# MrGreyPanda/NEM-MCMC-optimization

Hardware: AMD Instinct MI355X
Metric: order-score evals/sec (64 S-genes x 2000 effects); HBM GB/s fraction (higher is better)
Workload: dtype int8 fixed point 2^-38/ln2 + fp64 LSE

## Files before the change

### nem-mcmc-optimization_amd/csrc/nemo_factored_i8.hip

```cpp
#include "nemo_internal.h"

#include <math.h>

#include <string.h>

#include <algorithm>
#include <cmath>
#include <vector>

#ifndef NEMO_I8_ABLATE
#define NEMO_I8_ABLATE 0
#endif
#ifndef NEMO_I8L_RINIT
#define NEMO_I8L_RINIT 1
#endif
#ifndef NEMO_I8L_CINIT16
#define NEMO_I8L_CINIT16 1
#endif
#ifndef NEMO_I8L_PINGPONG
#define NEMO_I8L_PINGPONG 1
#endif
#ifndef NEMO_I8_WAVES_PER_SIMD
#define NEMO_I8_WAVES_PER_SIMD 2
#endif

namespace nemo {

namespace {

using i32x4 = __attribute__((ext_vector_type(4))) int;

constexpr double kPadG8 = -1.0e6;
constexpr int kARow = 6;
template <int ROWC>
__device__ __forceinline__ int a_byte(int i, int j) {
  if constexpr (ROWC == 4) return i * 64 + (((j >> 4) + 2 * ((i >> 2) & 3)) & 3) * 16 + (j & 15);
  else return i * (16 * ROWC) + j;
}

__device__ __forceinline__ double wsum(double v) {
#pragma unroll
  for (int o = 32; o >= 1; o >>= 1) v += __shfl_xor(v, o, kWave);
  return v;
}

__device__ __forceinline__ double exp_lse8(double x, const double* __restrict__ tab) {
  constexpr double kInvLn2x256 = 369.32993046757462707;
  constexpr double kLn2d256 = 2.7076061740622862e-03;
  constexpr double kMagic = 6755399441055744.0;
  const double t = fma(x, kInvLn2x256, kMagic);
  const double kf = t - kMagic;
  const int k = (int)(uint32_t)__builtin_bit_cast(uint64_t, t);
  const double r = fma(-kf, kLn2d256, x);
  double p = fma(r, 1.0 / 24.0, 1.0 / 6.0);
  p = fma(r, p, 0.5);
  p = fma(r, p, 1.0);
  p = fma(r, p, 1.0);
  return ldexp(p * tab[k & 255], k >> 8);
}

__device__ __forceinline__ double vmax8(double a, double b) {
  double r;
  asm("v_max_f64 %0, %1, %2" : "=v"(r) : "v"(a), "v"(b));
  return r;
}

__device__ __forceinline__ int xcd_index8(int L, int N, int remap) {
  if (!remap) return L;
  const int x = L & 7, k = L >> 3;
  const int q = N >> 3, r = N & 7;
  return x * q + (x < r ? x : r) + k;
}

struct EvalLds {
  i32x4* A;
  double* G;
  int* perm;
};

constexpr int kExpTabN = 2048;
constexpr int kTabBytes = kExpTabN * 8 + 128 * 16;

template <int SPAD, int NSL, int KH = 1, int NBUF = 1>
struct I8Lds {
  static constexpr int kElo = kTabBytes, kEhi = kElo + SPAD * 8, kBuf0 = kEhi + SPAD * 8;
  static constexpr int kG = 0, kGi = SPAD * 8, kPerm = kGi + 2 * SPAD * 4, kA = kPerm + SPAD * 4;
  static constexpr int kABytes = NSL * KH * SPAD * 64, kBuf = kA + kABytes, kImg = kBuf - kGi;
  static constexpr int kBytes = kBuf0 + NBUF * kBuf;
  static_assert((kBuf0 + kGi) % 16 == 0 && kA % 16 == 0 && kBuf % 16 == 0, "16-B alignment of gi and A");
  static_assert(NSL != 7 || KH != 1 || kImg == SPAD * kI8ImgRowBytes, "i8img_bytes follows this layout");

  static constexpr size_t bytes(size_t a_min = 0) {
    return (size_t)kBytes + (a_min > (size_t)kABytes ? a_min - kABytes : 0);
  }
  static __device__ __forceinline__ double2* ltab(double* lds) { return (double2*)((char*)lds + kExpTabN * 8); }
  static __device__ __forceinline__ double* elo(double* lds) { return (double*)((char*)lds + kElo); }
  static __device__ __forceinline__ double* ehi(double* lds) { return (double*)((char*)lds + kEhi); }
  static __device__ __forceinline__ EvalLds eval(double* lds, int k = 0) {
    char* p = (char*)lds + kBuf0 + k * kBuf;
    return EvalLds{(i32x4*)(p + kA), (double*)(p + kG), (int*)(p + kPerm)};
  }
  static __device__ __forceinline__ int* gi(double* lds, int k = 0) {
    return (int*)((char*)lds + kBuf0 + k * kBuf + kGi);
  }
};

template <int SPAD, int NSL, int ROWC = kARow>
__device__ __forceinline__ void i8_init_eval(EvalLds e, const int32_t* __restrict__ pb, int S, int tid,
                                             int nthreads, double padg = kPadG8) {
  for (int j = tid; j < S; j += nthreads) {
    int pj = pb[j];
    pj = pj < 0 ? 0 : (pj >= S ? S - 1 : pj);
    e.perm[pj] = j;
  }
  for (int i = tid; i < SPAD; i += nthreads) e.G[i] = i < S ? 0.0 : padg;
  for (int k = tid; k < NSL * SPAD * ROWC; k += nthreads) e.A[k] = i32x4{0, 0, 0, 0};
}

__device__ __forceinline__ int i8_npass(int S, int cap) {
  return (cap == 0 || cap >= S - 1) ? (S + 1) / 2 : S;
}

template <int WAVES>
__device__ __forceinline__ int i8_wave_passes(int S, int cap, int w) {
  const int npass = i8_npass(S, cap);
  return npass > w ? (npass - w + WAVES - 1) / WAVES : 0;
}

template <int SPAD, int NSL, int WAVES, int KB, int ROWC = kARow>
__device__ __forceinline__ void i8_prep_passes(EvalLds e, int k0, int w, int lane, int S, int cap,
                                               int cexp, const double* __restrict__ w01b,
                                               const double* __restrict__ elo_s,
                                               const double* __restrict__ ehi_s,
                                               const double2* __restrict__ ltab) {
  const bool packed = cap == 0 || cap >= S - 1;
  const int npass = packed ? (S + 1) / 2 : S;
  const int p = lane;
  int8_t* A8 = (int8_t*)e.A;
  int ii[KB], jj[KB];
  double sw[KB], ga[KB], gb[KB];
#pragma unroll
  for (int kk = 0; kk < KB; ++kk) {
    const int q = w + (k0 + kk) * WAVES;
    int qr = 0, pp = 0;
    bool act = false;
    if (q < npass) {
      if (packed) {
        const int q2 = S - 1 - q;
        if (p < q) { qr = q; pp = p; act = true; }
        else { qr = q2; pp = p - q; act = q2 != q && pp < q2; }
      } else {
        const int np = q < cap ? q : cap;
        qr = q; pp = q - 1 - p; act = p < np;
      }
    }
    ii[kk] = act ? e.perm[qr] : -1;
    jj[kk] = act ? e.perm[pp] : 0;
    sw[kk] = act ? w01b[ii[kk] * S + jj[kk]] : 0.0;
  }
#pragma unroll
  for (int kk = 0; kk < KB; ++kk) {
    const int q = w + (k0 + kk) * WAVES;
    const bool act = ii[kk] >= 0;
    double lo = 0.0;
    if (act && !(NEMO_I8_ABLATE & 8)) {
      const int i = ii[kk], j = jj[kk];
      const double s1 = 1.0 - sw[kk];
      lo = log_fast(fma(sw[kk], elo_s[j], s1), ltab);
      const double d = log_fast(fma(sw[kk], ehi_s[j], s1), ltab) - lo;
      double x = ldexp(d, 6 - cexp);
#pragma unroll
      for (int sl = 0; sl < NSL; ++sl) {
        const double qd = rint(x);
// ... 512 lines not shown
  constexpr int NP = 4;
  constexpr int NSL = 2 * NP;
  using L = I8Lds<SPAD, NSL>;
  extern __shared__ __attribute__((aligned(16))) double lds8[];
  const uint2* etab_o = (const uint2*)lds8;
  double2* ltab = L::ltab(lds8);
  double *elo_s = L::elo(lds8), *ehi_s = L::ehi(lds8);
  const EvalLds ev = L::eval(lds8);
  int* gi = L::gi(lds8);

  const I8Block blk = i8_block(nsets, split, remap);
  const int b = blk.b, s_begin = blk.s_begin, s_end = blk.s_end;
  const int tid = threadIdx.x;
  const int lane = tid & (kWave - 1);
  const int w = __builtin_amdgcn_readfirstlane(tid / kWave);
  const int col = lane & 15, rg = lane >> 4;

  i8_copy_tables<SPAD>(lds8, elo_s, ehi_s, tabs, e_lo, e_hi, S, tid, blockDim.x);
  i8_init_eval<SPAD, NSL, 4>(ev, pos + (size_t)b * S, S, tid, blockDim.x, padg);
  __syncthreads();
  if constexpr (DIAG) {
    int8_t* A8 = (int8_t*)ev.A;
    for (int k = tid; k < S * NSL; k += blockDim.x) {
      const int i = k / NSL, sl = k - i * NSL;
      A8[sl * SPAD * 64 + a_byte<4>(i, i)] = udig[k];
    }
  }
  for (int k0 = 0, my = i8_wave_passes<WAVES>(S, cap, w); k0 < my; k0 += 4)
    i8o_prep_passes<SPAD, WAVES, 4, 4>(ev, k0, w, lane, S, cap, cexp, w01 + (size_t)b * S * S, elo_s,
                                       ehi_s, ltab);
  __syncthreads();
  for (int i = tid; i < SPAD; i += blockDim.x) {
    const double g = DIAG && i < S ? ev.G[i] + u0[i] : ev.G[i];
    const double g0 = rint(ldexp(g, 24 - cexp));
    const double rho = fma(-g0, ldexp(1.0, cexp - 24), g);
    gi[i] = (int)g0;
    gi[SPAD + i] = (int)rint(ldexp(rho, 48 - cexp));
  }
  const uint32_t uln8 = (uint32_t)(4 * rg * E + col) * 8u;
  __syncthreads();
#if NEMO_I8_ABLATE & 32
  if (s_end > 0) return;
#endif

  const i32x4* Bt = (const i32x4*)B8;
  const i32x4* Gi = (const i32x4*)gi;
  const uint32_t a_lane = (uint32_t)(col * 4 + ((rg + 2 * (col >> 2)) & 3));
  int set = s_begin + w;
  if (set < s_end) {
    double lprod = 1.0;
    int lexp = 0;
    double uc[NR][4];
    int t = 8 * set;
    const __amdgpu_buffer_rsrc_t urs =
        __builtin_amdgcn_make_buffer_rsrc((void*)Uoff, (short)0, (int)((SPAD + 1) * E + 16) * 8, 0x00020000);
    auto uload = [&](int tt, int row) {
      return __builtin_bit_cast(double, __builtin_amdgcn_raw_buffer_load_b64(
                                            urs, uln8, (tt * 16 + row * E) * 8, 0));
    };
    if constexpr (!DIAG)
#pragma unroll
      for (int r = 0; r < NR; ++r)
#pragma unroll
        for (int g = 0; g < 4; ++g) uc[r][g] = uload(t, 16 * r + g);
    i32x4 bc = Bt[(size_t)t * kWave + lane];
    for (;;) {
      uint32_t ao = a_lane;
      asm volatile("" : "+v"(ao));
      const i32x4* Al = ev.A + ao;
      int tn = t + 1, setn = set;
      if (tn >= min(ntiles, 8 * set + 8)) {
        setn = set + WAVES;
        tn = 8 * setn;
      }
      const bool more = setn < s_end;
      const int tl = more ? tn : t;
      const i32x4 b1 = bc;
      const i32x4 b64 = b1 << 6;
      bc = Bt[(size_t)tl * kWave + lane];
      double ls0 = 0.0, ls1 = 0.0;
#pragma unroll
      for (int r = 0; r < NR; ++r) {
        i32x4 acc[NP];
        const i32x4 c0 = Gi[(16 * r) / 4 + rg];
        const i32x4 c1 = Gi[(SPAD + 16 * r) / 4 + rg];
#pragma unroll
        for (int pr = 0; pr < NP; ++pr) {
          const i32x4 a0 = Al[((2 * pr) * SPAD + 16 * r) * 4];
          const i32x4 a1 = Al[((2 * pr + 1) * SPAD + 16 * r) * 4];
          const i32x4 ci = pr == 1 ? c0 : (pr == 3 ? c1 : i32x4{0, 0, 0, 0});
          acc[pr] = __builtin_amdgcn_mfma_i32_16x16x64_i8(a0, b64, ci, 0, 0, 0);
          acc[pr] = __builtin_amdgcn_mfma_i32_16x16x64_i8(a1, b1, acc[pr], 0, 0, 0);
        }
#pragma unroll
        for (int g = 0; g < 4; ++g) {
          const int ta = (acc[0][g] << 12) + acc[1][g];
          const int tb = (acc[2][g] << 12) + acc[3][g];
          double x;
          if constexpr (DIAG) {
            x = fma((double)ta, sA, (double)tb * sB);
          } else {
            x = fma((double)ta, sA, fma((double)tb, sB, uc[r][g]));
            uc[r][g] = uload(tl, 16 * r + g);
          }
#if NEMO_I8_ABLATE & 1
          if (g & 1) ls1 += x;
          else ls0 += x;
#else
          if (g & 1) ls1 = exp_acc(x, etab_o, ls1);
          else ls0 = exp_acc(x, etab_o, ls0);
#endif
        }
      }
      i8_colprod(lprod, lexp, rowsum4(ls0 + ls1) + 1.0, t * 16 + col < E);
      if (setn != set) {
        double v = log(lprod) + (double)lexp * kLn2;
        v = wsum(lane < 16 ? v : 0.0);
        if (lane == 0) partial[(size_t)b * nsets + set] = nullsum[set] + v;
        lprod = 1.0;
        lexp = 0;
      }
      if (!more) break;
      t = tn;
      set = setn;
    }
  }
  if (split == 1) {
    __syncthreads();
    if (w == 0) {
      const double v = sum_partials(partial + (size_t)b * nsets, nsets, lane);
      if (lane == 0) ll_out[b] = v;
    }
  }
}

template <int NR, int WAVES, bool DIAG>
hipError_t launch_i8o_t(Ctx& c, int batch, int cap, const int32_t* d_pos, const double* d_w01,
                        double* d_ll, hipStream_t st, int* nparts, bool* finalized) {
  constexpr int SPAD = NR * 16;
  const int ntiles = (c.E + 15) / 16;
  const int nsets = (ntiles + 7) / 8;
  const int split = i8_split(256 * (NEMO_I8O_WAVES_PER_SIMD * 4 / WAVES), batch, nsets);
  const size_t lds = I8Lds<SPAD, 8>::bytes();
  const double sA = ldexp(1.0, c.i8_cexp - 24), sB = ldexp(1.0, c.i8_cexp - 48);
  score_i8o_kernel<NR, WAVES, DIAG><<<dim3(batch * split), WAVES * kWave, lds, st>>>(
      c.S, c.E, ntiles, nsets, split, cap, c.i8_cexp, c.i8o_padg, d_pos, d_w01, c.d_elo, c.d_ehi,
      c.d_B8, c.d_Uoff, c.d_udig, c.d_u0, c.d_nullsum, c.d_i8o_tabs, sA, sB, fpartial(c), d_ll,
      c.xcd_remap);
  *nparts = nsets;
  *finalized = split == 1;
  return hipGetLastError();
}

template <int NR, int WAVES, bool PP, class Hook>
__device__ __forceinline__ int i8l_walk2(const i32x4* __restrict__ Al0, const i32x4* __restrict__ Gi,
                                        const i32x4* __restrict__ Bt, const i32x4* __restrict__ Bt64,
                                        int set, int s_end, int ntiles, int E, int col, int lane,
                                        uint32_t a_lane, const double* __restrict__ nullsum,
                                        double* __restrict__ partial, size_t b, int nsets,
                                        const double2* __restrict__ ltab, Hook hook) {
  constexpr int SPAD = NR * 16;
  const int rg = lane >> 4;
  int it = 0;
  if (set < s_end) {
    double lprod = 1.0;
    int lexp = 0;
    int t = 8 * set;
    auto tend = [&](int st) { return min(ntiles, 8 * st + 8); };
    int t2 = t + 1 < tend(set) ? t + 1 : t;
    const __amdgpu_buffer_rsrc_t brs =
        __builtin_amdgcn_make_buffer_rsrc((void*)Bt, (short)0, 2 * ntiles * kWave * 16, 0x00020000);
    const uint32_t bln = (uint32_t)lane * 16u;
    auto bload = [&](int tile, int x64) {
      return __builtin_bit_cast(i32x4, __builtin_amdgcn_raw_buffer_load_b128(
                                           brs, bln, (x64 * ntiles + tile) * kWave * 16, 0));
    };
    i32x4 bca = bload(t, 0), bca64 = bload(t, 1);
    i32x4 bcb = bload(t2, 0), bcb64 = bload(t2, 1);
    auto iter = [&](const i32x4 b1a, const i32x4 b64a, const i32x4 b1b, const i32x4 b64b, i32x4& na,
                    i32x4& na64, i32x4& nb, i32x4& nb64) -> bool {
      uint32_t ao = a_lane;
      asm volatile("" : "+v"(ao));
      const i32x4* Al = Al0 + ao;
      const bool two = t2 != t;
      int tn = t + 2, setn = set;
      if (tn >= tend(set)) {
        setn = set + WAVES;
        tn = 8 * setn;
      }
      const bool more = setn < s_end;
      const int tla = __builtin_amdgcn_readfirstlane(more ? tn : t);
      const int tlb = __builtin_amdgcn_readfirstlane(more ? (tn + 1 < tend(setn) ? tn + 1 : tn) : t);
      na = bload(tla, 0);
      na64 = bload(tla, 1);
      nb = bload(tlb, 0);
      nb64 = bload(tlb, 1);
      double la0 = 0.0, la1 = 0.0, lb0 = 0.0, lb1 = 0.0;
#pragma unroll
      for (int r = 0; r < NR; ++r) {
        const i32x4 c0 = Gi[(16 * r) / 4 + rg];
        const i32x4 c1 = Gi[(SPAD + 16 * r) / 4 + rg];
        auto A = [&](int sl) { return Al[(sl * SPAD + 16 * r) * 4]; };
        i32x4 h0a, h0b, h1a, h1b, l0a, l0b, l1a, l1b;
        {
          const i32x4 a = A(0);
          h0a = __builtin_amdgcn_mfma_i32_16x16x64_i8(a, b64a, i32x4{0, 0, 0, 0}, 0, 0, 0);
          h0b = __builtin_amdgcn_mfma_i32_16x16x64_i8(a, b64b, i32x4{0, 0, 0, 0}, 0, 0, 0);
        }
        {
          const i32x4 a = A(1);
          h0a = __builtin_amdgcn_mfma_i32_16x16x64_i8(a, b1a, h0a, 0, 0, 0);
          h0b = __builtin_amdgcn_mfma_i32_16x16x64_i8(a, b1b, h0b, 0, 0, 0);
        }
        {
          const i32x4 a = A(2);
          h1a = __builtin_amdgcn_mfma_i32_16x16x64_i8(a, b64a, c0, 0, 0, 0);
          h1b = __builtin_amdgcn_mfma_i32_16x16x64_i8(a, b64b, c0, 0, 0, 0);
        }
        {
          const i32x4 a = A(3);
          h1a = __builtin_amdgcn_mfma_i32_16x16x64_i8(a, b1a, h1a, 0, 0, 0);
          h1b = __builtin_amdgcn_mfma_i32_16x16x64_i8(a, b1b, h1b, 0, 0, 0);
        }
#if NEMO_I8L_RINIT
        {
          const i32x4 a = A(5);
          l1a = __builtin_amdgcn_mfma_i32_16x16x64_i8(a, b64a, c1, 0, 0, 0);
          l1b = __builtin_amdgcn_mfma_i32_16x16x64_i8(a, b64b, c1, 0, 0, 0);
        }
        {
          const i32x4 a = A(6);
          l1a = __builtin_amdgcn_mfma_i32_16x16x64_i8(a, b1a, l1a, 0, 0, 0);
          l1b = __builtin_amdgcn_mfma_i32_16x16x64_i8(a, b1b, l1b, 0, 0, 0);
        }
        uint32_t t0a[4], t0b[4];
        uint64_t eva[4], evb[4];
        i32x4 ma, mb;
#pragma unroll
        for (int g = 0; g < 4; ++g) {
          t0a[g] = ((uint32_t)h0a[g] << 12) + (uint32_t)h1a[g];
          eva[g] = exp2_fx_load(t0a[g]);
          ma[g] = i8l_cinit16(t0a[g]);
        }
#pragma unroll
        for (int g = 0; g < 4; ++g) {
          t0b[g] = ((uint32_t)h0b[g] << 12) + (uint32_t)h1b[g];
          evb[g] = exp2_fx_load(t0b[g]);
          mb[g] = i8l_cinit16(t0b[g]);
        }
        {
          const i32x4 a = A(4);
          l0a = __builtin_amdgcn_mfma_i32_16x16x64_i8(a, b1a, ma, 0, 0, 0);
          l0b = __builtin_amdgcn_mfma_i32_16x16x64_i8(a, b1b, mb, 0, 0, 0);
        }
        auto epi = [&](const uint32_t (&t0)[4], const uint64_t (&evv)[4], const i32x4 l0, const i32x4 l1,
                       double& ls0, double& ls1) {
          double pr[4];
#pragma unroll
          for (int g = 0; g < 4; ++g) pr[g] = exp2_fx_series_r((int)(((uint32_t)l0[g] << 11) + (uint32_t)l1[g]));
#pragma unroll
          for (int g = 0; g < 4; ++g) {
            if (g & 1) ls1 = exp2_fx_apply(t0[g], evv[g], pr[g], ls1);
            else ls0 = exp2_fx_apply(t0[g], evv[g], pr[g], ls0);
          }
        };
        epi(t0a, eva, l0a, l1a, la0, la1);
        epi(t0b, evb, l0b, l1b, lb0, lb1);
#else
        {
          const i32x4 a = A(4);
          l0a = __builtin_amdgcn_mfma_i32_16x16x64_i8(a, b1a, i32x4{0, 0, 0, 0}, 0, 0, 0);
          l0b = __builtin_amdgcn_mfma_i32_16x16x64_i8(a, b1b, i32x4{0, 0, 0, 0}, 0, 0, 0);
        }
        {
          const i32x4 a = A(5);
          l1a = __builtin_amdgcn_mfma_i32_16x16x64_i8(a, b64a, c1, 0, 0, 0);
          l1b = __builtin_amdgcn_mfma_i32_16x16x64_i8(a, b64b, c1, 0, 0, 0);
        }
        {
          const i32x4 a = A(6);
          l1a = __builtin_amdgcn_mfma_i32_16x16x64_i8(a, b1a, l1a, 0, 0, 0);
          l1b = __builtin_amdgcn_mfma_i32_16x16x64_i8(a, b1b, l1b, 0, 0, 0);
        }
        auto epi = [&](const i32x4 h0, const i32x4 h1, const i32x4 l0, const i32x4 l1, double& ls0,
                       double& ls1) {
          uint32_t t0[4];
          uint64_t evv[4];
          double pr[4];
#pragma unroll
          for (int g = 0; g < 4; ++g) {
            t0[g] = ((uint32_t)h0[g] << 12) + (uint32_t)h1[g];
            evv[g] = exp2_fx_load(t0[g]);
          }
#pragma unroll
          for (int g = 0; g < 4; ++g)
            pr[g] = exp2_fx_series(t0[g], (int)(((uint32_t)l0[g] << 11) + (uint32_t)l1[g]));
#pragma unroll
          for (int g = 0; g < 4; ++g) {
            if (g & 1) ls1 = exp2_fx_apply(t0[g], evv[g], pr[g], ls1);
            else ls0 = exp2_fx_apply(t0[g], evv[g], pr[g], ls0);
          }
        };
        epi(h0a, h1a, l0a, l1a, la0, la1);
        epi(h0b, h1b, l0b, l1b, lb0, lb1);
#endif
      }
      const double l = rowsum_pair(la0 + la1, lb0 + lb1) + 1.0;
      const bool tb = (lane & 16) != 0;
      const bool ok = (((tb ? t2 : t) * 16 + col) < E) & (two | !tb);
      i8_colprod(lprod, lexp, l, ok);
      if (setn != set) {
        i8l_set_finish<true>(lprod, lexp, ltab, lane, nullsum, partial, b, nsets, set);
        lprod = 1.0;
        lexp = 0;
      }
      hook(it++);
      if (!more) return false;
      t = tn;
      t2 = tlb;
      set = setn;
      return true;
    };
    if constexpr (PP) {
      i32x4 bqa, bqa64, bqb, bqb64;
      for (;;) {
        if (!iter(bca, bca64, bcb, bcb64, bqa, bqa64, bqb, bqb64)) break;
        if (!iter(bqa, bqa64, bqb, bqb64, bca, bca64, bcb, bcb64)) break;
      }
    } else {
      for (;;) {
        i32x4 na, na64, nb, nb64;
        const bool more = iter(bca, bca64, bcb, bcb64, na, na64, nb, nb64);
        bca = na;
        bca64 = na64;
        bcb = nb;
        bcb64 = nb64;
        if (!more) break;
      }
    }
  }
  return it;
}

template <int NR, int WAVES, int OCC, int TT = 1, int MODE = 0>
__global__ __launch_bounds__(WAVES * kWave, OCC) void score_i8l_kernel(
    int S, int E, int ntiles, int nsets, int split, int cap, double padg,
    const int32_t* __restrict__ pos, const double* __restrict__ w01,
    const double* __restrict__ e_lo, const double* __restrict__ e_hi,
    const uint8_t* __restrict__ B8, const int8_t* __restrict__ udig, const double* __restrict__ u0,
    const double* __restrict__ nullsum, const void* __restrict__ tabs,
    double* __restrict__ partial, double* __restrict__ ll_out, int remap,
    int4* __restrict__ img = nullptr) {
  constexpr int SPAD = NR * 16;
  constexpr int NSL = 7;
  using L = I8Lds<SPAD, NSL>;
  extern __shared__ __attribute__((aligned(16))) double lds8[];
  double2* ltab = L::ltab(lds8);
  double *elo_s = L::elo(lds8), *ehi_s = L::ehi(lds8);
  const EvalLds ev = L::eval(lds8);
  int* gi = L::gi(lds8);

  const int work = xcd_index8((int)blockIdx.x, (int)gridDim.x, remap);
  const int b = work / split;
  const int part = work - b * split;
  const int spb = (nsets + split - 1) / split;
  const int s_begin = part * spb;
  const int s_end = min(nsets, s_begin + spb);
  const int tid = threadIdx.x;
  const int lane = tid & (kWave - 1);
  const int w = __builtin_amdgcn_readfirstlane(tid / kWave);
  const int col = lane & 15, rg = lane >> 4;

  constexpr int kImg4 = L::kImg / 16;
  {
    const int4* src = (const int4*)tabs;
    int4* dst = (int4*)lds8;
    for (int k = tid + (MODE == 1 ? kExpTabN * 8 / 16 : 0); k < kTabBytes / 16; k += blockDim.x)
      dst[k] = src[k];
    if constexpr (MODE != 2)
      for (int i = tid; i < SPAD; i += blockDim.x) {
        elo_s[i] = i < S ? e_lo[i] : 1.0;
        ehi_s[i] = i < S ? e_hi[i] : 1.0;
      }
  }
  if constexpr (MODE == 2) {
    const int4* src = img + (size_t)b * kImg4;
    int4* dst = (int4*)gi;
    for (int k = tid; k < kImg4; k += blockDim.x) dst[k] = src[k];
    __syncthreads();
  } else {
    i8_init_eval<SPAD, NSL, 4>(ev, pos + (size_t)b * S, S, tid, blockDim.x, padg);
    __syncthreads();
    i8l_diag<SPAD>(ev.A, udig, S, tid, blockDim.x);
    for (int k0 = 0, my = i8_wave_passes<WAVES>(S, cap, w); k0 < my; k0 += 4)
      i8o_prep_passes<SPAD, WAVES, 4, 4, true>(ev, k0, w, lane, S, cap, 0, w01 + (size_t)b * S * S, elo_s,
                                               ehi_s, ltab);
    __syncthreads();
    i8l_split_g<SPAD>(ev, gi, u0, S, tid, blockDim.x);
    __syncthreads();
    if constexpr (MODE == 1) {
      const int4* src = (const int4*)gi;
      int4* dst = img + (size_t)b * kImg4;
      for (int k = tid; k < kImg4; k += blockDim.x) dst[k] = src[k];
      return;
    }
  }
#if NEMO_I8_ABLATE & 32
  if (s_end > 0) return;
#endif

  const i32x4* Bt = (const i32x4*)B8;
  const i32x4* Bt64 = Bt + (size_t)ntiles * kWave;
  const i32x4* Gi = (const i32x4*)gi;
  const uint32_t a_lane = (uint32_t)(col * 4 + ((rg + 2 * (col >> 2)) & 3));
  int set = s_begin + w;
  if constexpr (TT == 1) {
    int set = s_begin + w;
    if (set < s_end) {
      double lprod = 1.0;
      int lexp = 0;
      int t = 8 * set;
      i32x4 bc = Bt[(size_t)t * kWave + lane];
      i32x4 bc64 = Bt64[(size_t)t * kWave + lane];
      for (;;) {
        uint32_t ao = a_lane;
        asm volatile("" : "+v"(ao));
        const i32x4* Al = ev.A + ao;
        int tn = t + 1, setn = set;
        if (tn >= min(ntiles, 8 * set + 8)) {
          setn = set + WAVES;
          tn = 8 * setn;
        }
        const bool more = setn < s_end;
        const int tl = more ? tn : t;
        const i32x4 b1 = bc, b64 = bc64;
        bc = Bt[(size_t)tl * kWave + lane];
        bc64 = Bt64[(size_t)tl * kWave + lane];
        double ls0 = 0.0, ls1 = 0.0;
  #pragma unroll
        for (int r = 0; r < NR; ++r) {
          const i32x4 c0 = Gi[(16 * r) / 4 + rg];
          const i32x4 c1 = Gi[(SPAD + 16 * r) / 4 + rg];
  #if NEMO_I8_ABLATE & 128
          auto A = [&](int sl) { return Al[((sl & ~1) * SPAD + 16 * r) * 4]; };
  #else
          auto A = [&](int sl) { return Al[(sl * SPAD + 16 * r) * 4]; };
  #endif
  #if NEMO_I8_ABLATE & 2
          const i32x4 h0 = A(0) + A(1) + b64, h1 = A(2) + A(3) + c0, l0 = A(4) + b1,
                      l1 = A(5) + A(6) + c1;
  #else
          i32x4 h0 = __builtin_amdgcn_mfma_i32_16x16x64_i8(A(0), b64, i32x4{0, 0, 0, 0}, 0, 0, 0);
          h0 = __builtin_amdgcn_mfma_i32_16x16x64_i8(A(1), b1, h0, 0, 0, 0);
          i32x4 h1 = __builtin_amdgcn_mfma_i32_16x16x64_i8(A(2), b64, c0, 0, 0, 0);
          h1 = __builtin_amdgcn_mfma_i32_16x16x64_i8(A(3), b1, h1, 0, 0, 0);
          const i32x4 l0 = __builtin_amdgcn_mfma_i32_16x16x64_i8(A(4), b1, i32x4{0, 0, 0, 0}, 0, 0, 0);
          i32x4 l1 = __builtin_amdgcn_mfma_i32_16x16x64_i8(A(5), b64, c1, 0, 0, 0);
          l1 = __builtin_amdgcn_mfma_i32_16x16x64_i8(A(6), b1, l1, 0, 0, 0);
  #endif
          uint32_t t0[4];
          uint64_t evv[4];
          double pr[4];
#pragma unroll
          for (int g = 0; g < 4; ++g) {
            t0[g] = ((uint32_t)h0[g] << 12) + (uint32_t)h1[g];
            evv[g] = exp2_fx_load(t0[g]);
          }
#pragma unroll
          for (int g = 0; g < 4; ++g)
            pr[g] = exp2_fx_series(t0[g], (int)(((uint32_t)l0[g] << 11) + (uint32_t)l1[g]));
#pragma unroll
          for (int g = 0; g < 4; ++g) {
            if (g & 1) ls1 = exp2_fx_apply(t0[g], evv[g], pr[g], ls1);
            else ls0 = exp2_fx_apply(t0[g], evv[g], pr[g], ls0);
          }
        }
        i8_colprod(lprod, lexp, rowsum4(ls0 + ls1) + 1.0, t * 16 + col < E);
        if (setn != set) {
          i8l_set_finish<false>(lprod, lexp, ltab, lane, nullsum, partial, b, nsets, set);
          lprod = 1.0;
          lexp = 0;
        }
        if (!more) break;
        t = tn;
        set = setn;
      }
    }
  } else {
    i8l_walk2<NR, WAVES, NEMO_I8L_PINGPONG != 0>(ev.A, Gi, Bt, Bt64, set, s_end, ntiles, E, col, lane, a_lane,
                                                 nullsum, partial, b, nsets, ltab, [](int) {});
  }
  if (split == 1) {
    __syncthreads();
    if (w == 0) {
      const double v = sum_partials(partial + (size_t)b * nsets, nsets, lane);
      if (lane == 0) ll_out[b] = v;
    }
  }
}

constexpr size_t kI8sColsum = 16384;

template <int NR>
__global__ __launch_bounds__(8 * kWave, NEMO_I8O_WAVES_PER_SIMD) void score_i8s_kernel(
    int S, int E, int ntiles, int nsets, int split, int cap, double padg,
    const int32_t* __restrict__ pos, const double* __restrict__ w01,
    const double* __restrict__ e_lo, const double* __restrict__ e_hi,
    const uint8_t* __restrict__ B8, const int8_t* __restrict__ udig, const double* __restrict__ u0,
    const double* __restrict__ nullsum, const void* __restrict__ tabs,
    double* __restrict__ partial, double* __restrict__ ll_out, int remap) {
  constexpr int WAVES = 8;
  constexpr int SPAD = NR * 16;
  constexpr int NSL = 7;
  constexpr int NG = WAVES / NR;
  using L = I8Lds<SPAD, NSL>;
  extern __shared__ __attribute__((aligned(16))) double lds8[];
  double2* ltab = L::ltab(lds8);
  double *elo_s = L::elo(lds8), *ehi_s = L::ehi(lds8);
  const EvalLds ev = L::eval(lds8);
  int* gi = L::gi(lds8);
  double* colsum = (double*)ev.A;

  const I8Block blk = i8_block(nsets, split, remap);
  const int b = blk.b, s_begin = blk.s_begin, s_end = blk.s_end;
  const int tid = threadIdx.x;
  const int lane = tid & (kWave - 1);
  const int w = __builtin_amdgcn_readfirstlane(tid / kWave);
  const int rb = w % NR, grp = w / NR;
  const int col = lane & 15, rg = lane >> 4;

  i8_copy_tables<SPAD>(lds8, elo_s, ehi_s, tabs, e_lo, e_hi, S, tid, blockDim.x);
  i8_init_eval<SPAD, NSL, 4>(ev, pos + (size_t)b * S, S, tid, blockDim.x, padg);
  __syncthreads();
  i8l_diag<SPAD>(ev.A, udig, S, tid, blockDim.x);
  for (int k0 = 0, my = i8_wave_passes<WAVES>(S, cap, w); k0 < my; k0 += 4)
    i8o_prep_passes<SPAD, WAVES, 4, 4, true>(ev, k0, w, lane, S, cap, 0, w01 + (size_t)b * S * S, elo_s,
                                             ehi_s, ltab);
  __syncthreads();
  i8l_split_g<SPAD>(ev, gi, u0, S, tid, blockDim.x);
  __syncthreads();
  i32x4 af[NSL];
  {
    const i32x4* Al = ev.A + (uint32_t)(col * 4 + ((rg + 2 * (col >> 2)) & 3));
#pragma unroll
    for (int sl = 0; sl < NSL; ++sl) af[sl] = Al[(sl * SPAD + 16 * rb) * 4];
  }
  const i32x4 c0 = ((const i32x4*)gi)[(16 * rb) / 4 + rg];
  const i32x4 c1 = ((const i32x4*)gi)[(SPAD + 16 * rb) / 4 + rg];
  __syncthreads();
#if NEMO_I8_ABLATE & 32
  if (s_end > 0) return;
#endif

  const i32x4* Bt = (const i32x4*)B8;
  const int nsb = s_end > s_begin ? s_end - s_begin : 0;
  const int niter = (nsb + NG - 1) / NG;
  int tpre = 8 * (s_begin + grp);
  i32x4 bc = Bt[(size_t)min(tpre, ntiles - 1) * kWave + lane];
  for (int k = 0; k < niter; ++k) {
    const int set = s_begin + k * NG + grp;
    double* cs = colsum + (size_t)((grp * 2 + (k & 1)) * 8) * NR * 16;
    if (set < s_end) {
      const int t_end = min(ntiles, 8 * set + 8);
      for (int t = 8 * set; t < t_end; ++t) {
        const int tn = t + 1 < t_end ? t + 1 : 8 * (set + NG);
        const i32x4 b1 = bc;
        const i32x4 b64 = b1 << 6;
        bc = Bt[(size_t)min(tn, ntiles - 1) * kWave + lane];
        const i32x4 h0 = __builtin_amdgcn_mfma_i32_16x16x64_i8(
            af[1], b1, __builtin_amdgcn_mfma_i32_16x16x64_i8(af[0], b64, i32x4{0, 0, 0, 0}, 0, 0, 0), 0, 0, 0);
        const i32x4 h1 = __builtin_amdgcn_mfma_i32_16x16x64_i8(
            af[3], b1, __builtin_amdgcn_mfma_i32_16x16x64_i8(af[2], b64, c0, 0, 0, 0), 0, 0, 0);
        const i32x4 l0 = __builtin_amdgcn_mfma_i32_16x16x64_i8(af[4], b1, i32x4{0, 0, 0, 0}, 0, 0, 0);
        const i32x4 l1 = __builtin_amdgcn_mfma_i32_16x16x64_i8(
            af[6], b1, __builtin_amdgcn_mfma_i32_16x16x64_i8(af[5], b64, c1, 0, 0, 0), 0, 0, 0);
        double ls0 = 0.0, ls1 = 0.0;
        uint32_t t0[4];
        uint64_t evt[4];
        double pr[4];
#pragma unroll
        for (int g = 0; g < 4; ++g) {
          t0[g] = ((uint32_t)h0[g] << 12) + (uint32_t)h1[g];
          evt[g] = exp2_fx_load(t0[g]);
        }
#pragma unroll
        for (int g = 0; g < 4; ++g)
          pr[g] = exp2_fx_series(t0[g], (int)(((uint32_t)l0[g] << 11) + (uint32_t)l1[g]));
#pragma unroll
        for (int g = 0; g < 4; ++g) {
          if (g & 1) ls1 = exp2_fx_apply(t0[g], evt[g], pr[g], ls1);
          else ls0 = exp2_fx_apply(t0[g], evt[g], pr[g], ls0);
        }
        const double v = rowsum4(ls0 + ls1);
        if (lane < 16) cs[((t - 8 * set) * NR + rb) * 16 + col] = v;
      }
    }
    __syncthreads();
    if (set < s_end && rb == k % NR) {
      double lp = 1.0;
      int le = 0;
#pragma unroll
      for (int h = 0; h < 2; ++h) {
        const int tt = (lane >> 4) + 4 * h;
        const int t = 8 * set + tt;
        double l = 1.0;
#pragma unroll
        for (int q = 0; q < NR; ++q) l += cs[(tt * NR + q) * 16 + col];
        i8_colprod(lp, le, l, t < ntiles && t * 16 + col < E);
      }
      const double v = wsum(log(lp) + (double)le * kLn2);
      if (lane == 0) partial[(size_t)b * nsets + set] = nullsum[set] + v;
    }
  }
  if (split == 1) {
    __syncthreads();
    if (w == 0) {
      const double v = sum_partials(partial + (size_t)b * nsets, nsets, lane);
      if (lane == 0) ll_out[b] = v;
    }
  }
}

template <int NR, int WAVES>
__global__ __launch_bounds__(WAVES * kWave, NEMO_I8L2_OCC) void score_i8p_kernel(
    int S, int E, int ntiles, int nsets, int batch, int cap, double padg,
    const int32_t* __restrict__ pos, const double* __restrict__ w01,
    const double* __restrict__ e_lo, const double* __restrict__ e_hi,
    const uint8_t* __restrict__ B8, const int8_t* __restrict__ udig, const double* __restrict__ u0,
    const double* __restrict__ nullsum, const void* __restrict__ tabs,
    double* __restrict__ partial, double* __restrict__ ll_out) {
  constexpr int SPAD = NR * 16;
  constexpr int NSL = 7;
  constexpr int kBufG = 0, kBufGi = SPAD * 8, kBufPerm = kBufGi + 2 * SPAD * 4, kBufA = kBufPerm + SPAD * 4;
  constexpr int kBuf = kBufA + NSL * SPAD * 64;
  static_assert(kBuf == I8Lds<SPAD, NSL, 1, 2>::kBuf && kBufA == I8Lds<SPAD, NSL>::kA, "I8Lds describes it");
  extern __shared__ __attribute__((aligned(16))) double lds8[];
  uint2* etab_o = (uint2*)lds8;
  double2* ltab = (double2*)(etab_o + kExpTabN);
  double* elo_s = (double*)(ltab + 128);
  double* ehi_s = elo_s + SPAD;
  char* bufs = (char*)(ehi_s + SPAD);
  auto evb = [&](int k) {
    EvalLds e;
    char* p = bufs + k * kBuf;
    e.G = (double*)(p + kBufG);
    e.perm = (int*)(p + kBufPerm);
    e.A = (i32x4*)(p + kBufA);
    return e;
  };
  auto gib = [&](int k) { return (int*)(bufs + k * kBuf + kBufGi); };

  const int tid = threadIdx.x;
  const int lane = tid & (kWave - 1);
  const int w = __builtin_amdgcn_readfirstlane(tid / kWave);
  const int col = lane & 15, rg = lane >> 4;
  const int nb = gridDim.x;
  const int b0 = blockIdx.x;
  if (b0 >= batch) return;

  auto set_perm = [&](int k, int e) {
    int* perm = evb(k).perm;
    for (int j = tid; j < S; j += blockDim.x) {
      int pj = pos[(size_t)e * S + j];
      pj = pj < 0 ? 0 : (pj >= S ? S - 1 : pj);
      perm[pj] = j;
    }
  };
  auto zero_a = [&](int k) {
    i32x4* A = evb(k).A;
    for (int q = tid; q < NSL * SPAD * 4; q += blockDim.x) A[q] = i32x4{0, 0, 0, 0};
  };
  auto diag = [&](int k) {
    int8_t* A8 = (int8_t*)evb(k).A;
    for (int q = tid; q < S * NSL; q += blockDim.x) {
      const int i = q / NSL, sl = q - i * NSL;
      const int8_t d = udig[i * 8 + sl];
      A8[sl * SPAD * 64 + a_byte<4>(i, i)] = sl == 4 ? (int8_t)(2 * d) : d;
    }
  };
  auto prep = [&](int k, int e) {
    constexpr int KB = 4;
    const int npass = i8_npass(S, cap);
    const int my = npass > w ? (npass - w + WAVES - 1) / WAVES : 0;
    for (int k0 = 0; k0 < my; k0 += KB)
      i8o_prep_passes<SPAD, WAVES, KB, 4, true>(evb(k), k0, w, lane, S, cap, 0, w01 + (size_t)e * S * S,
                                                elo_s, ehi_s, ltab);
  };
  auto finalize_g = [&](int k) {
    const EvalLds ev = evb(k);
    int* gi = gib(k);
    for (int i = tid; i < SPAD; i += blockDim.x) {
      const double g = i < S ? ev.G[i] + u0[i] : ev.G[i];
      const double g0 = rint(g * kL2Scale);
      gi[i] = (int)g0 + (1023 << 20);
      gi[SPAD + i] = (int)rint(fma(g, kL2Scale, -g0) * 262144.0);
    }
  };

  {
    const int4* src = (const int4*)tabs;
    int4* dst = (int4*)lds8;
    for (int k = tid; k < (kExpTabN * 8 + 128 * 16) / 16; k += blockDim.x) dst[k] = src[k];
    for (int i = tid; i < SPAD; i += blockDim.x) {
      elo_s[i] = i < S ? e_lo[i] : 1.0;
      ehi_s[i] = i < S ? e_hi[i] : 1.0;
    }
  }
  for (int k = 0; k < 2; ++k) {
    for (int i = tid; i < SPAD; i += blockDim.x) evb(k).G[i] = i < S ? 0.0 : padg;
    zero_a(k);
  }
  set_perm(0, b0);
  if (b0 + nb < batch) set_perm(1, b0 + nb);
  __syncthreads();
  diag(0);
  diag(1);
  __syncthreads();
  prep(0, b0);
  __syncthreads();
  finalize_g(0);
  __syncthreads();

  const i32x4* Bt = (const i32x4*)B8;
  const i32x4* Bt64 = Bt + (size_t)ntiles * kWave;
  const uint32_t a_lane = (uint32_t)(col * 4 + ((rg + 2 * (col >> 2)) & 3));
  int k = 0;
  for (int e = b0; e < batch; e += nb, k ^= 1) {
    const int en = e + nb;
    bool pending = en < batch;
    i8l_walk2<NR, WAVES, false>(evb(k).A, (const i32x4*)gib(k), Bt, Bt64, w, nsets, ntiles, E, col, lane, a_lane,
                         nullsum, partial, (size_t)e, nsets, ltab, [&](int it) {
                           if (pending && it == 0) {
                             prep(k ^ 1, en);
                             pending = false;
                           }
                         });
    if (pending) prep(k ^ 1, en);
    __syncthreads();
    if (w == 0) {
      const double v = sum_partials(partial + (size_t)e * nsets, nsets, lane);
      if (lane == 0) ll_out[e] = v;
    }
    if (en < batch) finalize_g(k ^ 1);
    const bool again = en + nb < batch;
    if (again) {
      zero_a(k);
      set_perm(k, en + nb);
    }
    __syncthreads();
    if (again) diag(k);
  }
}

template <int NR>
hipError_t launch_i8s_t(Ctx& c, int batch, int cap, const int32_t* d_pos, const double* d_w01,
                        double* d_ll, hipStream_t st, int* nparts, bool* finalized) {
  constexpr int SPAD = NR * 16;
  const int ntiles = (c.E + 15) / 16;
  const int nsets = (ntiles + 7) / 8;
  const int split = i8_split(256 * (NEMO_I8O_WAVES_PER_SIMD * 4 / 8), batch, nsets);
  const size_t lds = I8Lds<SPAD, 7>::bytes(kI8sColsum);
  score_i8s_kernel<NR><<<dim3(batch * split), 8 * kWave, lds, st>>>(
      c.S, c.E, ntiles, nsets, split, cap, c.i8o_padg, d_pos, d_w01, c.d_elo, c.d_ehi, c.d_B8,
      c.d_udig2, c.d_u0, c.d_nullsum, c.d_i8o_tabs, fpartial(c), d_ll, c.xcd_remap);
  *nparts = nsets;
  *finalized = split == 1;
  return hipGetLastError();
}

template <int NR>
hipError_t launch_i8p_t(Ctx& c, int batch, int cap, const int32_t* d_pos, const double* d_w01,
                        double* d_ll, hipStream_t st, int* nparts, bool* finalized) {
  constexpr int SPAD = NR * 16;
  const int ntiles = (c.E + 15) / 16;
  const int nsets = (ntiles + 7) / 8;
  const size_t lds = I8Lds<SPAD, 7, 1, 2>::kBytes;
  int dev = 0, ncu = 0;
  hipError_t ge = hipGetDevice(&dev);
  if (ge == hipSuccess) ge = hipDeviceGetAttribute(&ncu, hipDeviceAttributeMultiprocessorCount, dev);
  if (ge != hipSuccess) return ge;
  if (ncu <= 0) ncu = 256;
  if (lds > 65536) {
    hipError_t ae = hipFuncSetAttribute((const void*)score_i8p_kernel<NR, 8>,
                                        hipFuncAttributeMaxDynamicSharedMemorySize, (int)lds);
    if (ae != hipSuccess) return ae;
  }
  const int grid = std::min(batch, 3 * ncu);
  score_i8p_kernel<NR, 8><<<dim3(grid), 8 * kWave, lds, st>>>(
      c.S, c.E, ntiles, nsets, batch, cap, c.i8o_padg, d_pos, d_w01, c.d_elo, c.d_ehi, c.d_B8,
      c.d_udig2, c.d_u0, c.d_nullsum, c.d_i8o_tabs, fpartial(c), d_ll);
  *nparts = nsets;
  *finalized = true;
  return hipGetLastError();
}

template <int NR, int WAVES, int OCC = NEMO_I8O_WAVES_PER_SIMD, int TT = 1, bool SPLIT = false>
hipError_t launch_i8l_t(Ctx& c, int batch, int cap, const int32_t* d_pos, const double* d_w01,
                        double* d_ll, hipStream_t st, int* nparts, bool* finalized) {
  using L = I8Lds<NR * 16, 7>;
  const int ntiles = (c.E + 15) / 16;
  const int nsets = (ntiles + 7) / 8;
  const int split = i8_split(256 * (OCC * 4 / WAVES), batch, nsets);
  const size_t lds = L::bytes();
  if constexpr (SPLIT) {
    if (!c.d_i8img || c.i8img_cap < batch || (size_t)L::kImg != i8img_bytes(c.fspad))
      return hipErrorInvalidValue;
    score_i8l_kernel<NR, WAVES, OCC, TT, 1><<<dim3(batch), WAVES * kWave, lds, st>>>(
        c.S, c.E, ntiles, nsets, 1, cap, c.i8o_padg, d_pos, d_w01, c.d_elo, c.d_ehi, c.d_B8,
        c.d_udig2, c.d_u0, c.d_nullsum, c.d_i8o_tabs, fpartial(c), d_ll, c.xcd_remap, (int4*)c.d_i8img);
    score_i8l_kernel<NR, WAVES, OCC, TT, 2><<<dim3(batch * split), WAVES * kWave, lds, st>>>(
        c.S, c.E, ntiles, nsets, split, cap, c.i8o_padg, d_pos, d_w01, c.d_elo, c.d_ehi, c.d_B8,
        c.d_udig2, c.d_u0, c.d_nullsum, c.d_i8o_tabs, fpartial(c), d_ll, c.xcd_remap, (int4*)c.d_i8img);
  } else {
    score_i8l_kernel<NR, WAVES, OCC, TT><<<dim3(batch * split), WAVES * kWave, lds, st>>>(
        c.S, c.E, ntiles, nsets, split, cap, c.i8o_padg, d_pos, d_w01, c.d_elo, c.d_ehi, c.d_B8,
        c.d_udig2, c.d_u0, c.d_nullsum, c.d_i8o_tabs, fpartial(c), d_ll, c.xcd_remap);
  }
  *nparts = nsets;
  *finalized = split == 1;
  return hipGetLastError();
}

constexpr int kWideKH = 2;

__device__ __forceinline__ void i8w_digits(int8_t* A8, int i, int j, double d) {
  constexpr int SPAD = 128, SL = SPAD * 64;
  const double hd = rint(d * kL2Scale);
  const int h = (int)hd;
  const int l = (int)rint(fma(d, kL2Scale, -hd) * 262144.0);
  const int off = (j >> 6) * SL + a_byte<4>(i, j & 63);
  const int hb = h + 32 * (1 + 64 + 4096), lb = l + 32 * (1 + 64);
  A8[(0 * kWideKH) * SL + off] = (int8_t)(hb >> 18);
  A8[(1 * kWideKH) * SL + off] = (int8_t)(((hb >> 12) & 63) - 32);
  A8[(2 * kWideKH) * SL + off] = (int8_t)(((hb >> 6) & 63) - 32);
  A8[(3 * kWideKH) * SL + off] = (int8_t)((hb & 63) - 32);
  A8[(4 * kWideKH) * SL + off] = (int8_t)(2 * (lb >> 12));
  A8[(5 * kWideKH) * SL + off] = (int8_t)(((lb >> 6) & 63) - 32);
  A8[(6 * kWideKH) * SL + off] = (int8_t)((lb & 63) - 32);
}

template <int WAVES, int KB>
__device__ __forceinline__ void i8w_prep_passes(EvalLds e, int k0, int w, int lane, int S, int cap,
                                                const double* __restrict__ w01b,
                                                const double* __restrict__ elo_s,
                                                const double* __restrict__ ehi_s,
                                                const double2* __restrict__ ltab) {
  const bool packed = cap == 0 || cap >= S - 1;
  const int npass = packed ? (S + 1) / 2 : S;
  int8_t* A8 = (int8_t*)e.A;
  double ga[KB], gb[KB];
#pragma unroll
  for (int kk = 0; kk < KB; ++kk) {
    ga[kk] = 0.0;
    gb[kk] = 0.0;
    const int q = w + (k0 + kk) * WAVES;
#pragma unroll
    for (int hr = 0; hr < kWideKH; ++hr) {
      const int p = lane + 64 * hr;
      int qr = 0, pp = 0;
      bool act = false, side_a = true;
      if (q < npass) {
        if (packed) {
          const int q2 = S - 1 - q;
          if (p < q) { qr = q; pp = p; act = true; }
          else { qr = q2; pp = p - q; act = q2 != q && pp < q2; side_a = false; }
        } else {
          const int np = q < cap ? q : cap;
          qr = q; pp = q - 1 - p; act = p < np;
        }
      }
      if (act) {
        const int i = e.perm[qr], j = e.perm[pp];
        const double sw = w01b[i * S + j];
        const double s1 = 1.0 - sw;
        const double lo = log_fast(fma(sw, elo_s[j], s1), ltab);
        const double d = log_fast(fma(sw, ehi_s[j], s1), ltab) - lo;
        i8w_digits(A8, i, j, d);
        if (side_a) ga[kk] += lo;
        else gb[kk] += lo;
      }
    }
  }
#pragma unroll
// ... 471 lines not shown
```

Baseline: 14.06 million.

## Software-pipeline LDS A-fragment loads across row blocks with explicit sched barriers

Adds a scheduled variant of the int8 row-block loop that preloads the next row's A and G fragments from LDS into registers while the current row's exp2 series and apply math runs. sched_barrier fences and register pinning fix the order of the MFMA, exponent-table, and accumulate phases. The next tile's B buffer loads are pushed to the last row block. The aim is to hide LDS and global latency behind MFMA and VALU work, at the cost of higher register pressure and fixed scheduling that could hurt occupancy. The variant is on by default when NR > 1.

```diff
diff --git a/nem-mcmc-optimization_amd/csrc/nemo_factored_i8.hip b/nem-mcmc-optimization_amd/csrc/nemo_factored_i8.hip
--- a/nem-mcmc-optimization_amd/csrc/nemo_factored_i8.hip
+++ b/nem-mcmc-optimization_amd/csrc/nemo_factored_i8.hip
@@ -19,6 +19,9 @@
 #endif
 #ifndef NEMO_I8L_PINGPONG
 #define NEMO_I8L_PINGPONG 1
+#endif
+#ifndef NEMO_I8L_SCHED
+#define NEMO_I8L_SCHED 1
 #endif
 #ifndef NEMO_I8_WAVES_PER_SIMD
 #define NEMO_I8_WAVES_PER_SIMD 2
@@ -837,7 +840,7 @@
   return hipGetLastError();
 }
 
-template <int NR, int WAVES, bool PP, class Hook>
+template <int NR, int WAVES, bool PP, bool SCHED, class Hook>
 __device__ __forceinline__ int i8l_walk2(const i32x4* __restrict__ Al0, const i32x4* __restrict__ Gi,
                                         const i32x4* __restrict__ Bt, const i32x4* __restrict__ Bt64,
                                         int set, int s_end, int ntiles, int E, int col, int lane,
@@ -862,6 +865,88 @@
     };
     i32x4 bca = bload(t, 0), bca64 = bload(t, 1);
     i32x4 bcb = bload(t2, 0), bcb64 = bload(t2, 1);
+    i32x4 fa[7], fc0, fc1;
+    auto request_hi = [&](const i32x4* Al, int r) {
+#pragma unroll
+      for (int sl = 0; sl < 4; ++sl) fa[sl] = Al[(sl * SPAD + 16 * r) * 4];
+      fc0 = Gi[(16 * r) / 4 + rg];
+    };
+    auto request_lo = [&](const i32x4* Al, int r) {
+#pragma unroll
+      for (int sl = 4; sl < 7; ++sl) fa[sl] = Al[(sl * SPAD + 16 * r) * 4];
+      fc1 = Gi[(SPAD + 16 * r) / 4 + rg];
+    };
+    if constexpr (SCHED) {
+      request_hi(Al0 + a_lane, 0);
+      request_lo(Al0 + a_lane, 0);
+    }
+    auto pin = [](i32x4& v) { asm volatile("" : "+v"(v)); };
+    auto i8l_rowblocks_sched = [&](const i32x4 b1a, const i32x4 b64a, const i32x4 b1b, const i32x4 b64b,
+                                   const i32x4* Al, double& la0, double& la1, double& lb0, double& lb1,
+                                   auto&& bprefetch) {
+#pragma unroll
+      for (int r = 0; r < NR; ++r) {
+        if (r == NR - 1) bprefetch();
+        const i32x4 z = i32x4{0, 0, 0, 0};
+        i32x4 h0a = __builtin_amdgcn_mfma_i32_16x16x64_i8(fa[0], b64a, z, 0, 0, 0);
+        i32x4 h0b = __builtin_amdgcn_mfma_i32_16x16x64_i8(fa[0], b64b, z, 0, 0, 0);
+        h0a = __builtin_amdgcn_mfma_i32_16x16x64_i8(fa[1], b1a, h0a, 0, 0, 0);
+        h0b = __builtin_amdgcn_mfma_i32_16x16x64_i8(fa[1], b1b, h0b, 0, 0, 0);
+        i32x4 h1a = __builtin_amdgcn_mfma_i32_16x16x64_i8(fa[2], b64a, fc0, 0, 0, 0);
+        i32x4 h1b = __builtin_amdgcn_mfma_i32_16x16x64_i8(fa[2], b64b, fc0, 0, 0, 0);
+        h1a = __builtin_amdgcn_mfma_i32_16x16x64_i8(fa[3], b1a, h1a, 0, 0, 0);
+        h1b = __builtin_amdgcn_mfma_i32_16x16x64_i8(fa[3], b1b, h1b, 0, 0, 0);
+        i32x4 l1a = __builtin_amdgcn_mfma_i32_16x16x64_i8(fa[5], b64a, fc1, 0, 0, 0);
+        i32x4 l1b = __builtin_amdgcn_mfma_i32_16x16x64_i8(fa[5], b64b, fc1, 0, 0, 0);
+        l1a = __builtin_amdgcn_mfma_i32_16x16x64_i8(fa[6], b1a, l1a, 0, 0, 0);
+        l1b = __builtin_amdgcn_mfma_i32_16x16x64_i8(fa[6], b1b, l1b, 0, 0, 0);
+        pin(h0a), pin(h0b), pin(h1a), pin(h1b), pin(l1a), pin(l1b);
+        __builtin_amdgcn_sched_barrier(0);
+        uint32_t t0a[4], t0b[4];
+        i32x4 ma, mb;
+#pragma unroll
+        for (int g = 0; g < 4; ++g) {
+          t0a[g] = ((uint32_t)h0a[g] << 12) + (uint32_t)h1a[g];
+          ma[g] = i8l_cinit16(t0a[g]);
+        }
+#pragma unroll
+        for (int g = 0; g < 4; ++g) {
+          t0b[g] = ((uint32_t)h0b[g] << 12) + (uint32_t)h1b[g];
+          mb[g] = i8l_cinit16(t0b[g]);
+        }
+        i32x4 l0a = __builtin_amdgcn_mfma_i32_16x16x64_i8(fa[4], b1a, ma, 0, 0, 0);
+        i32x4 l0b = __builtin_amdgcn_mfma_i32_16x16x64_i8(fa[4], b1b, mb, 0, 0, 0);
+        pin(l0a), pin(l0b);
+        __builtin_amdgcn_sched_barrier(0);
+        uint64_t eva[4], evb[4];
+#pragma unroll
+        for (int g = 0; g < 4; ++g) eva[g] = exp2_fx_load(t0a[g]);
+#pragma unroll
+        for (int g = 0; g < 4; ++g) evb[g] = exp2_fx_load(t0b[g]);
+        __builtin_amdgcn_sched_barrier(0);
+        request_hi(Al, r + 1 < NR ? r + 1 : 0);
+        __builtin_amdgcn_sched_barrier(0);
+        double pa[4], pb[4];
+#pragma unroll
+        for (int g = 0; g < 4; ++g) pa[g] = exp2_fx_series_r((int)(((uint32_t)l0a[g] << 11) + (uint32_t)l1a[g]));
+#pragma unroll
+        for (int g = 0; g < 4; ++g) pb[g] = exp2_fx_series_r((int)(((uint32_t)l0b[g] << 11) + (uint32_t)l1b[g]));
+        __builtin_amdgcn_sched_barrier(0);
+        request_lo(Al, r + 1 < NR ? r + 1 : 0);
+        __builtin_amdgcn_sched_barrier(0);
+#pragma unroll
+        for (int g = 0; g < 4; ++g) {
+          if (g & 1) la1 = exp2_fx_apply(t0a[g], eva[g], pa[g], la1);
+          else la0 = exp2_fx_apply(t0a[g], eva[g], pa[g], la0);
+        }
+#pragma unroll
+        for (int g = 0; g < 4; ++g) {
+          if (g & 1) lb1 = exp2_fx_apply(t0b[g], evb[g], pb[g], lb1);
+          else lb0 = exp2_fx_apply(t0b[g], evb[g], pb[g], lb0);
+        }
+        __builtin_amdgcn_sched_barrier(0);
+      }
+    };
     auto iter = [&](const i32x4 b1a, const i32x4 b64a, const i32x4 b1b, const i32x4 b64b, i32x4& na,
                     i32x4& na64, i32x4& nb, i32x4& nb64) -> bool {
       uint32_t ao = a_lane;
@@ -876,11 +961,21 @@
       const bool more = setn < s_end;
       const int tla = __builtin_amdgcn_readfirstlane(more ? tn : t);
       const int tlb = __builtin_amdgcn_readfirstlane(more ? (tn + 1 < tend(setn) ? tn + 1 : tn) : t);
-      na = bload(tla, 0);
-      na64 = bload(tla, 1);
-      nb = bload(tlb, 0);
-      nb64 = bload(tlb, 1);
+      if constexpr (!SCHED) {
+        na = bload(tla, 0);
+        na64 = bload(tla, 1);
+        nb = bload(tlb, 0);
+        nb64 = bload(tlb, 1);
+      }
       double la0 = 0.0, la1 = 0.0, lb0 = 0.0, lb1 = 0.0;
+      if constexpr (SCHED) {
+        i8l_rowblocks_sched(b1a, b64a, b1b, b64b, Al, la0, la1, lb0, lb1, [&] {
+          na = bload(tla, 0);
+          na64 = bload(tla, 1);
+          nb = bload(tlb, 0);
+          nb64 = bload(tlb, 1);
+        });
+      } else
 #pragma unroll
       for (int r = 0; r < NR; ++r) {
         const i32x4 c0 = Gi[(16 * r) / 4 + rg];
@@ -1172,8 +1267,9 @@
       }
     }
   } else {
-    i8l_walk2<NR, WAVES, NEMO_I8L_PINGPONG != 0>(ev.A, Gi, Bt, Bt64, set, s_end, ntiles, E, col, lane, a_lane,
-                                                 nullsum, partial, b, nsets, ltab, [](int) {});
+    constexpr bool kSched = NEMO_I8L_SCHED != 0 && NEMO_I8L_RINIT != 0 && NR > 1;
+    i8l_walk2<NR, WAVES, NEMO_I8L_PINGPONG != 0, kSched>(ev.A, Gi, Bt, Bt64, set, s_end, ntiles, E, col, lane,
+                                                         a_lane, nullsum, partial, b, nsets, ltab, [](int) {});
   }
   if (split == 1) {
     __syncthreads();
@@ -1413,7 +1509,7 @@
   for (int e = b0; e < batch; e += nb, k ^= 1) {
     const int en = e + nb;
     bool pending = en < batch;
-    i8l_walk2<NR, WAVES, false>(evb(k).A, (const i32x4*)gib(k), Bt, Bt64, w, nsets, ntiles, E, col, lane, a_lane,
+    i8l_walk2<NR, WAVES, false, false>(evb(k).A, (const i32x4*)gib(k), Bt, Bt64, w, nsets, ntiles, E, col, lane, a_lane,
                          nullsum, partial, (size_t)e, nsets, ltab, [&](int it) {
                            if (pending && it == 0) {
                              prep(k ^ 1, en);
```

Measured after the change: 14.39 million (median of 6 runs). +2.4%, better.
